# nilsfriess/ParMGMC

Measured on AMD Instinct MI355X. Metric: Gaussian samples/sec on 512^3 3D DMDA (7-pt Laplacian precision, red-black Gibbs sweep = 1 sorgibbs sample), higher is better.
Workload: dtype f64

## Files before the change

### parmgmc_amd/csrc/kernels_grid.hip

```cpp
#include <hip/hip_runtime.h>
#include <cstring>
#include <stdlib.h>
#include "pmg_kernels.h"
#define PMG_RNG_TU grid
#include "pmg_rng.hpp"

namespace {

typedef double d2 __attribute__((ext_vector_type(2)));

__device__ __forceinline__ d2 ld2(const double *p) { return *reinterpret_cast<const d2 *>(p); }

__device__ __forceinline__ d2 ld2_sys(const double *p)
{
  const unsigned long long a = __hip_atomic_load(reinterpret_cast<const unsigned long long *>(p), __ATOMIC_RELAXED, __HIP_MEMORY_SCOPE_SYSTEM);
  const unsigned long long b = __hip_atomic_load(reinterpret_cast<const unsigned long long *>(p) + 1, __ATOMIC_RELAXED, __HIP_MEMORY_SCOPE_SYSTEM);
  d2                       v;
  v.x = __longlong_as_double((long long)a);
  v.y = __longlong_as_double((long long)b);
  return v;
}
__device__ __forceinline__ void st2_sys(double *p, d2 v)
{
  __hip_atomic_store(reinterpret_cast<unsigned long long *>(p), (unsigned long long)__double_as_longlong(v.x), __ATOMIC_RELAXED, __HIP_MEMORY_SCOPE_SYSTEM);
  __hip_atomic_store(reinterpret_cast<unsigned long long *>(p) + 1, (unsigned long long)__double_as_longlong(v.y), __ATOMIC_RELAXED, __HIP_MEMORY_SCOPE_SYSTEM);
}

__device__ __forceinline__ const double *at_bytes(const double *base, uint32_t byte_off) { return reinterpret_cast<const double *>(reinterpret_cast<const char *>(base) + byte_off); }
__device__ __forceinline__ double       *at_bytes(double *base, uint32_t byte_off) { return reinterpret_cast<double *>(reinterpret_cast<char *>(base) + byte_off); }

__device__ __forceinline__ double uniform(double v)
{
  return __hiloint2double(__builtin_amdgcn_readfirstlane(__double2hiint(v)), __builtin_amdgcn_readfirstlane(__double2loint(v)));
}

template <bool PACKED>
__device__ __forceinline__ double table_at(const double (&a)[8], int idx)
{
  if (!PACKED) return uniform(a[idx]);
  double v = a[1];
  v        = idx == 2 ? a[2] : v;
  v        = idx == 3 ? a[3] : v;
  v        = idx == 4 ? a[4] : v;
  v        = idx == 5 ? a[5] : v;
  v        = idx == 6 ? a[6] : v;
  return v;
}

__device__ __forceinline__ void wave_wait_flag(const uint64_t *f, uint64_t v, unsigned *err, unsigned long long *spin_total)
{
  if (threadIdx.x == 0) {
    unsigned long long spins = 0;
    while (__hip_atomic_load(f, __ATOMIC_RELAXED, __HIP_MEMORY_SCOPE_SYSTEM) < v) {
      __builtin_amdgcn_s_sleep(8);
      ++spins;
      if ((spins & 0xFFFFu) == 0 && err && __hip_atomic_load(err, __ATOMIC_RELAXED, __HIP_MEMORY_SCOPE_SYSTEM)) break;
      if (spins > (1ull << 28)) {
        if (err) {
          err[1] = 0x10u;
          err[2] = (unsigned)v;
          err[3] = (unsigned)__hip_atomic_load(f, __ATOMIC_RELAXED, __HIP_MEMORY_SCOPE_SYSTEM);
          __hip_atomic_store(err, 1u, __ATOMIC_RELAXED, __HIP_MEMORY_SCOPE_SYSTEM);
        }
        break;
      }
    }
    if (spins && spin_total) atomicAdd(spin_total, spins);
  }
  __builtin_amdgcn_fence(__ATOMIC_ACQUIRE, "workgroup");
}

template <bool NOISY, bool OMEGA1, bool HALO, bool PACKED>
__device__ __forceinline__ void grid_color_sweep_body(const pmgk_grid_layout &L, const pmgk_grid_op &op, int c, int t, int j, int k, pmg::LogTabEntry *tab, pmg::LogTabEntry tab_entry, const pmgk_grid_halo &halo, const double *__restrict__ b_own, const double *__restrict__ y_other, double *__restrict__ y_own)
{
  const int kg = k + L.kz0;
  bool live = j < L.ny && 2 * t < L.sx && 4 * t + ((c + j + kg) & 1) < L.nx;
  if (NOISY) {
    if (!__builtin_amdgcn_ballot_w64(live)) return;
    t = live ? t : 0;
    if (PACKED) j = live ? j : 0;
  } else if (!live)
    return;
  const int p  = (c + j + kg) & 1;
  const int i0 = 4 * t + p, i1 = i0 + 2;
  const bool v1 = i1 < L.nx;

  const bool    hasS = j > 0, hasN = j < L.ny - 1, hasD = kg > 0, hasU = kg < L.nzg - 1;
  const double  h2 = op.h2;
  const int64_t  rowoff = (int64_t)(k + 1) * L.sp + (int64_t)j * L.sx;
  const uint32_t lo     = 16u * (uint32_t)t;
  const double  *yo_row = y_other + rowoff;
  const int    eo = p ? (2 * t + 2 < L.sx ? 2 : 1) : (t > 0 ? -1 : 0);
  const bool   hasW0 = i0 > 0, hasE0 = i0 < L.nx - 1, hasE1 = i1 < L.nx - 1;
  const int    nyz = PACKED ? (int)hasS + (int)hasN + (int)hasD + (int)hasU : min(j, 1) + min(L.ny - 1 - j, 1) + min(kg, 1) + min(L.nzg - 1 - kg, 1);
  const bool   two0 = hasW0 && hasE0, two1 = hasE1;
  const double idA = table_at<PACKED>(op.idiag, nyz + 1), idB = table_at<PACKED>(op.idiag, nyz + 2);
  const double sqA = NOISY ? table_at<PACKED>(op.sqrtdiag, nyz + 1) : 0.0, sqB = NOISY ? table_at<PACKED>(op.sqrtdiag, nyz + 2) : 0.0;
  double      *out_row = y_own + rowoff;
  d2     Vc = ld2(at_bytes(yo_row, lo));
  double ed = *at_bytes(yo_row, lo + 8u * (uint32_t)eo);
  d2     oS = ld2(at_bytes(yo_row - (hasS ? L.sx : 0), lo));
  d2     oN = ld2(at_bytes(yo_row + (hasN ? L.sx : 0), lo));
  const int64_t inplane = (int64_t)j * L.sx + 2 * t;
  d2      oD = (HALO && k == 0 && halo.glo) ? ld2_sys(halo.glo + inplane) : ld2(at_bytes(yo_row - (hasD ? L.sp : 0), lo));
  d2      oU = (HALO && k == L.nz - 1 && halo.ghi) ? ld2_sys(halo.ghi + inplane) : ld2(at_bytes(yo_row + (hasU ? L.sp : 0), lo));
#ifndef PMG_GRID_NO_NT
  d2     bb = __builtin_nontemporal_load(reinterpret_cast<const d2 *>(at_bytes(b_own + rowoff, lo)));
#else
  d2     bb = ld2(at_bytes(b_own + rowoff, lo));
#endif
  pmg::RngConsts K;
  if (NOISY) {
    __builtin_amdgcn_sched_barrier(0);
    K = pmg::load_sincos_consts();
    __builtin_amdgcn_sched_barrier(0);
  }

  double z0 = 0.0, z1 = 0.0;
  if (NOISY) {
    pmg::normal_pair_fill((uint32_t)t, (uint32_t)(j + (int64_t)L.ny * kg), (uint32_t)op.sweep, ((uint32_t)(op.sweep >> 32) & 0x7fffffffu) | ((uint32_t)c << 31), op.key0, op.key1, tab_entry, tab, (int)threadIdx.x, K, z0, z1);
    asm volatile("" : "+v"(Vc.x), "+v"(Vc.y), "+v"(ed), "+v"(oS.x), "+v"(oS.y), "+v"(oN.x), "+v"(oN.y), "+v"(oD.x), "+v"(oD.y), "+v"(oU.x), "+v"(oU.y), "+v"(bb.x), "+v"(bb.y) : "v"(z0), "v"(z1));
  }
  const double L0 = p ? Vc.x : ed, R0 = p ? Vc.y : Vc.x, L1 = R0, R1 = p ? ed : Vc.y;
  const double idg0 = two0 ? idB : idA, idg1 = two1 ? idB : idA;
  const double hS = hasS ? h2 : 0.0, hN = hasN ? h2 : 0.0, hD = hasD ? h2 : 0.0, hU = hasU ? h2 : 0.0;

  double w0 = bb.x, w1 = bb.y;
  if (NOISY) {
    const double sq0 = two0 ? sqB : sqA, sq1 = two1 ? sqB : sqA;
    w0 = z0 * sq0 + bb.x;
    w1 = z1 * sq1 + bb.y;
  }
  double s0 = w0, s1 = w1;
  s0 = s0 + hD * oD.x;
  s1 = s1 + hD * oD.y;
  s0 = s0 + hS * oS.x;
  s1 = s1 + hS * oS.y;
  s0 = s0 + (hasW0 ? h2 : 0.0) * L0;
  s1 = s1 + h2 * L1;
  s0 = s0 + (hasE0 ? h2 : 0.0) * R0;
  s1 = s1 + (hasE1 ? h2 : 0.0) * R1;
  s0 = s0 + hN * oN.x;
  s1 = s1 + hN * oN.y;
  s0 = s0 + hU * oU.x;
  s1 = s1 + hU * oU.y;

  double r0, r1;
  if (OMEGA1) {
    r0 = idg0 * s0;
    r1 = idg1 * s1;
  } else {
    const d2 yo2 = ld2(at_bytes(out_row, lo));
    r0           = op.one_minus_omega * yo2.x + idg0 * s0;
    r1           = op.one_minus_omega * yo2.y + idg1 * s1;
  }
  const d2 out = {r0, v1 ? r1 : 0.0};
  if (NOISY) {
    asm volatile("" ::"v"(out.x), "v"(out.y), "s"(out_row));
    if (!live) return;
  }
#ifndef PMG_GRID_NO_NT
  __builtin_nontemporal_store(out, reinterpret_cast<d2 *>(at_bytes(out_row, lo)));
#else
  *reinterpret_cast<d2 *>(at_bytes(out_row, lo)) = out;
#endif
  if (HALO) {
    if (k == 0 && halo.plo) st2_sys(halo.plo + inplane, out);
    if (k == L.nz - 1 && halo.phi) st2_sys(halo.phi + inplane, out);
  }
}

template <bool NOISY, bool OMEGA1>
__device__ __forceinline__ d2 grid_row_update(const pmgk_grid_op &op, int p, bool hasW0, bool hasE0, bool hasE1, bool v1, bool hasS, bool hasN, bool hasD, bool hasU, double h2, bool two0, bool two1, double idA, double idB, double sqA, double sqB, d2 Vc, double ed, d2 oS, d2 oN, d2 oD, d2 oU, d2 bb, double z0, double z1, const double *out_row, uint32_t lo)
{
  const double L0 = p ? Vc.x : ed, R0 = p ? Vc.y : Vc.x, L1 = R0, R1 = p ? ed : Vc.y;
  const double idg0 = two0 ? idB : idA, idg1 = two1 ? idB : idA;
  const double hS = hasS ? h2 : 0.0, hN = hasN ? h2 : 0.0, hD = hasD ? h2 : 0.0, hU = hasU ? h2 : 0.0;

  double w0 = bb.x, w1 = bb.y;
  if (NOISY) {
    const double sq0 = two0 ? sqB : sqA, sq1 = two1 ? sqB : sqA;
    w0 = z0 * sq0 + bb.x;
    w1 = z1 * sq1 + bb.y;
  }
  double s0 = w0, s1 = w1;
  s0 = s0 + hD * oD.x;
  s1 = s1 + hD * oD.y;
  s0 = s0 + hS * oS.x;
  s1 = s1 + hS * oS.y;
  s0 = s0 + (hasW0 ? h2 : 0.0) * L0;
  s1 = s1 + h2 * L1;
  s0 = s0 + (hasE0 ? h2 : 0.0) * R0;
  s1 = s1 + (hasE1 ? h2 : 0.0) * R1;
  s0 = s0 + hN * oN.x;
  s1 = s1 + hN * oN.y;
  s0 = s0 + hU * oU.x;
  s1 = s1 + hU * oU.y;

  double r0, r1;
  if (OMEGA1) {
    r0 = idg0 * s0;
    r1 = idg1 * s1;
  } else {
    const d2 yo2 = ld2(at_bytes(out_row, lo));
    r0           = op.one_minus_omega * yo2.x + idg0 * s0;
    r1           = op.one_minus_omega * yo2.y + idg1 * s1;
  }
  const d2 out = {r0, v1 ? r1 : 0.0};
  return out;
}

template <bool PACKED>
__device__ __forceinline__ void grid_thread_position(int nbx, int bandw, int ty, int &t, int &j)
{
  if (PACKED) {
    const int flat = ((int)blockIdx.x * 4 + ty) * 64 + (int)threadIdx.x;
    j              = flat / nbx;
    t              = flat - j * nbx;
  } else {
    const int bx = bandw > 0 ? (int)(blockIdx.x >> 3) : (int)blockIdx.x;
    const int jl = (int)blockIdx.y * 4 + ty;
    t            = bx * 64 + threadIdx.x;
    j            = bandw > 0 ? (jl < bandw ? (int)(blockIdx.x & 7u) * bandw + jl : 0x40000000) : jl;
  }
}

template <bool NOISY, bool OMEGA1, bool HALO, bool PACKED, bool TAIL>
__global__ __launch_bounds__(256) __attribute__((amdgpu_num_sgpr(96))) void grid_color_sweep_kernel(pmgk_grid_layout L, pmgk_grid_op op, int c, int nbx, int zmain, int bandw, int kbegin, int kstride, int kcount, int tmain, int tailw, pmgk_grid_halo halo, const double *__restrict__ b_own, const double *__restrict__ y_other, double *__restrict__ y_own)
{
  const int ty = __builtin_amdgcn_readfirstlane(threadIdx.y);
  __shared__ pmg::LogTabEntry s_logtab[NOISY ? 4 * PMG_LOGTAB_SIZE : 1];
  pmg::LogTabEntry           *tab = s_logtab + (NOISY ? ty * PMG_LOGTAB_SIZE : 0);
  pmg::LogTabEntry            tab_entry = {0.0, 0.0};
  if (NOISY) {
    const d2 e = ld2(reinterpret_cast<const double *>(pmg::g_logtab + threadIdx.x));
    tab_entry  = {e.x, e.y};
  }
  int                         t, j;
  const int                   zsplit = zmain > 0 ? zmain : kcount;
  if (TAIL && (int)blockIdx.z >= zsplit) {
    const int tb  = (int)blockIdx.x + (int)gridDim.x * ((int)blockIdx.y + (int)gridDim.y * ((int)blockIdx.z - zsplit));
    const bool compact = tailw == 1 && L.nx == 4 * tmain + 1 && (L.sx & 15) != 0;
    const int  slots   = compact ? (L.ny + 1) / 2 : L.ny * tailw;
    const int  per     = (slots + 255) / 256;
    const int  kz = tb / per, part = tb - kz * per;
    if (kz >= kcount) return;
    const int f = (part * 4 + ty) * 64 + (int)threadIdx.x, kt = kbegin + kz * kstride;
    if (compact) {
      j = 2 * f + ((c + kt + L.kz0) & 1);
      t = tmain;
    } else {
      j = f / tailw;
      t = tmain + f - j * tailw;
    }
    grid_color_sweep_body<NOISY, OMEGA1, false, true>(L, op, c, t, j, kt, tab, tab_entry, halo, b_own, y_other, y_own);
    return;
  }
  grid_thread_position<PACKED>(nbx, bandw, ty, t, j);

  int k = kbegin + (int)blockIdx.z * kstride;
  if (!HALO && !PACKED && zmain > 0) {
    const int xcd = (int)(blockIdx.x & 7u), extra = max(xcd - (8 - (L.ny - 8 * bandw)), 0);
    const int first = xcd * bandw + extra, nl = bandw + (xcd >= 8 - (L.ny - 8 * bandw) ? 1 : 0);
    const int w     = ((int)blockIdx.y + (int)gridDim.y * (int)blockIdx.z) * 4 + ty;
    if (nl <= 0) return;
    const int kz = w / nl;
    if (kz >= kcount) return;
    t = (int)(blockIdx.x >> 3) * 64 + (int)threadIdx.x;
    j = first + (w - kz * nl);
    k = kbegin + kz * kstride;
  }
  if (HALO && halo.full) {
    const int z = (int)blockIdx.z;
    k           = z == 0 ? 0 : (z == 1 ? L.nz - 1 : z - 1);
    const bool face_lo = k == 0, face_hi = k == L.nz - 1;
    if (face_lo && halo.wlo) wave_wait_flag(halo.wlo, halo.wval, halo.err, halo.spins);
    if (face_hi && halo.whi) wave_wait_flag(halo.whi, halo.wval, halo.err, halo.spins);
    grid_color_sweep_body<NOISY, OMEGA1, HALO, PACKED>(L, op, c, t, j, k, tab, tab_entry, halo, b_own, y_other, y_own);
    if (face_lo || face_hi) {
      asm volatile("s_waitcnt vmcnt(0)" ::: "memory");
      __builtin_amdgcn_fence(__ATOMIC_RELEASE, "workgroup");
      __syncthreads();
      if (threadIdx.x == 0 && threadIdx.y == 0) {
        const unsigned nface  = L.nz > 1 ? 2u : 1u;
        const unsigned expect = gridDim.x * gridDim.y * nface;
        if (atomicAdd(halo.counter, 1u) == expect - 1u) {
          *halo.counter = 0;
          if (halo.slo) __hip_atomic_store(halo.slo, halo.sval, __ATOMIC_RELAXED, __HIP_MEMORY_SCOPE_SYSTEM);
          if (halo.shi) __hip_atomic_store(halo.shi, halo.sval, __ATOMIC_RELAXED, __HIP_MEMORY_SCOPE_SYSTEM);
        }
      }
    }
    return;
  }
  grid_color_sweep_body<NOISY, OMEGA1, HALO, PACKED>(L, op, c, t, j, k, tab, tab_entry, halo, b_own, y_other, y_own);
}

struct grid_pair_launch {
  int32_t  nx, ny, sx, kz0, nzg;
  int32_t  c, kbegin, kcount, npair;
  int32_t  bandw;
  int32_t  flat;
  int32_t  thr;
  uint32_t mul0, mul1;
  uint32_t sp8, sx8;
};

template <bool OMEGA1>
__global__ __launch_bounds__(256) __attribute__((amdgpu_num_sgpr(96), amdgpu_waves_per_eu(4, 4))) void grid_color_pair_sweep_kernel(grid_pair_launch P, const double *__restrict__ b_own, const double *__restrict__ y_other, double *__restrict__ y_own, pmgk_grid_op op)
{
  const int ty = __builtin_amdgcn_readfirstlane(threadIdx.y);
  __shared__ pmg::LogTabEntry s_logtab[4 * PMG_LOGTAB_SIZE];
  pmg::LogTabEntry           *tab       = s_logtab + ty * PMG_LOGTAB_SIZE;
  const d2                    tab_e     = ld2(reinterpret_cast<const double *>(pmg::g_logtab + threadIdx.x));
  const pmg::LogTabEntry      tab_entry = {tab_e.x, tab_e.y};
  asm volatile("" ::"s"(P.sp8), "s"(P.sx8), "s"(b_own), "s"(y_other), "s"(op.key0), "s"(op.key1), "s"(op.sweep));
  const int xcd = (int)(blockIdx.x & 7u);
  int       bx, j, kz;
  if (P.flat) {
    const int  over  = xcd - P.thr;
    const int  first = xcd * P.bandw + max(over, 0), nl = P.bandw + (over >= 0 ? 1 : 0);
    const int  w     = ((int)blockIdx.y * 4 + P.flat * (int)blockIdx.z) + ty;
    kz = (int)__umulhi((uint32_t)w, over >= 0 ? P.mul1 : P.mul0);
    bx = (int)(blockIdx.x >> 3);
    j  = first + (w - kz * nl);
  } else {
    const int jl = (int)blockIdx.y * 4 + ty;
    bx = P.bandw > 0 ? (int)(blockIdx.x >> 3) : (int)blockIdx.x;
    j  = P.bandw > 0 ? (jl < P.bandw ? xcd * P.bandw + jl : 0x40000000) : jl;
    kz = (int)blockIdx.z;
  }
  if (j >= P.ny || kz >= P.npair) return;

  const bool pair = 2 * kz + 1 < P.kcount;
  const int  k0 = P.kbegin + 2 * kz, kg0 = k0 + P.kz0, kg1 = kg0 + (pair ? 1 : 0);
  const int  p0 = (P.c + j + kg0) & 1, p1 = (P.c + j + kg1) & 1;
  int        t  = bx * 64 + (int)threadIdx.x;
  const bool inrow = 2 * t < P.sx, live0 = inrow && 4 * t + p0 < P.nx, live1 = pair && inrow && 4 * t + p1 < P.nx;
  const bool live = live0 || live1;
  if (!__builtin_amdgcn_ballot_w64(live)) return;
  t = live ? t : 0;
  const bool hasS = j > 0, hasN = j < P.ny - 1, hasD0 = kg0 > 0, hasU0 = kg0 < P.nzg - 1, hasU1 = kg1 < P.nzg - 1;
  const uint32_t sp8 = P.sp8, sx8 = P.sx8, dS = hasS ? sx8 : 0u, dN = hasN ? sx8 : 0u;
  const uint32_t d0 = sp8, d1 = sp8 + (pair ? sp8 : 0u);
  const uint64_t rowm = (uint64_t)(uint32_t)k0 * sp8 + (uint32_t)j * sx8;
  const char    *yo   = reinterpret_cast<const char *>(y_other) + rowm, *bo = reinterpret_cast<const char *>(b_own) + rowm;
  const uint32_t lo   = 16u * (uint32_t)t;
  const uint32_t v0 = lo + d0, v1 = lo + d1;
  const uint32_t eW = t > 0 ? (uint32_t)-8 : 0u, eE = 2 * t + 2 < P.sx ? 16u : 8u;
  const uint32_t m0 = (uint32_t)-p0, m1 = (uint32_t)-p1;
  const uint32_t e0 = (eE & m0) | (eW & ~m0), e1 = (eE & m1) | (eW & ~m1);
  const double *yod = reinterpret_cast<const double *>(yo), *bod = reinterpret_cast<const double *>(bo);
  d2     rA  = ld2(at_bytes(yod, lo + (hasD0 ? 0u : sp8)));
  d2     rB  = ld2(at_bytes(yod, v0));
  d2     rC  = ld2(at_bytes(yod, v0 + (hasU0 ? sp8 : 0u)));
  d2     rE  = ld2(at_bytes(yod, v1 + (hasU1 ? sp8 : 0u)));
  double ed0 = *at_bytes(yod, v0 + e0);
  double ed1 = *at_bytes(yod, v1 + e1);
  d2     oS0 = ld2(at_bytes(yod, lo + (d0 - dS)));
  d2     oN0 = ld2(at_bytes(yod, lo + (d0 + dN)));
  d2     oS1 = ld2(at_bytes(yod, lo + (d1 - dS)));
  d2     oN1 = ld2(at_bytes(yod, lo + (d1 + dN)));
#ifndef PMG_GRID_NO_NT
  d2     bb0 = __builtin_nontemporal_load(reinterpret_cast<const d2 *>(at_bytes(bod, v0)));
  d2     bb1 = __builtin_nontemporal_load(reinterpret_cast<const d2 *>(at_bytes(bod, v1)));
#else
  d2     bb0 = ld2(at_bytes(bod, v0));
  d2     bb1 = ld2(at_bytes(bod, v1));
#endif
  __builtin_amdgcn_sched_barrier(0);
  int      jr = j, kr0 = kg0, kr1 = kg1;
  uint32_t key0 = op.key0, key1 = op.key1, sweep_lo = (uint32_t)op.sweep, sweep_hi = (uint32_t)(op.sweep >> 32);
  asm volatile("" : "+s"(jr), "+s"(kr0), "+s"(kr1), "+s"(key0), "+s"(key1), "+s"(sweep_lo), "+s"(sweep_hi));
  const pmg::RngConsts K = pmg::load_sincos_consts();
  const int      nyz0 = min(jr, 1) + min(P.ny - 1 - jr, 1) + min(kr0, 1) + min(P.nzg - 1 - kr0, 1);
  const int      nyz1 = min(jr, 1) + min(P.ny - 1 - jr, 1) + min(kr1, 1) + min(P.nzg - 1 - kr1, 1);
  const double   idA0 = uniform(op.idiag[nyz0 + 1]), idB0 = uniform(op.idiag[nyz0 + 2]), idA1 = uniform(op.idiag[nyz1 + 1]), idB1 = uniform(op.idiag[nyz1 + 2]);
  const double   sqA0 = uniform(op.sqrtdiag[nyz0 + 1]), sqB0 = uniform(op.sqrtdiag[nyz0 + 2]);
  const double   sqA1 = uniform(op.sqrtdiag[nyz1 + 1]), sqB1 = uniform(op.sqrtdiag[nyz1 + 2]);
  double        *out = reinterpret_cast<double *>(reinterpret_cast<char *>(y_own) + rowm);
  __builtin_amdgcn_sched_barrier(0);
  double z00, z01, z10, z11;
  pmg::normal_pair_fill2((uint32_t)t, (uint32_t)(jr + (int64_t)P.ny * kr0), (uint32_t)(jr + (int64_t)P.ny * kr1), sweep_lo, (sweep_hi & 0x7fffffffu) | ((uint32_t)P.c << 31), key0, key1, tab_entry, tab, (int)threadIdx.x, K, z00, z01, z10, z11);
  asm volatile("" : "+v"(rA.x), "+v"(rA.y), "+v"(rB.x), "+v"(rB.y), "+v"(rC.x), "+v"(rC.y), "+v"(rE.x), "+v"(rE.y), "+v"(ed0), "+v"(ed1) : "v"(z00), "v"(z01), "v"(z10), "v"(z11));
  asm volatile("" : "+v"(oS0.x), "+v"(oS0.y), "+v"(oN0.x), "+v"(oN0.y), "+v"(oS1.x), "+v"(oS1.y), "+v"(oN1.x), "+v"(oN1.y), "+v"(bb0.x), "+v"(bb0.y), "+v"(bb1.x), "+v"(bb1.y) : "v"(z00), "v"(z01), "v"(z10), "v"(z11));
  int    tr = t;
  double h2 = op.h2;
  asm volatile("" : "+v"(tr), "+s"(h2), "+s"(jr), "+s"(kr0), "+s"(kr1) : "v"(z00), "v"(z01), "v"(z10), "v"(z11));
  const bool uS = jr > 0, uN = jr < P.ny - 1, uD0 = kr0 > 0, uU0 = kr0 < P.nzg - 1, uD1 = kr1 > 0, uU1 = kr1 < P.nzg - 1;
  const int  q0 = (P.c + jr + kr0) & 1, q1 = (P.c + jr + kr1) & 1;
  const int  i00 = 4 * tr + q0, i01 = i00 + 2, i10 = 4 * tr + q1, i11 = i10 + 2;
  const bool hasW00 = i00 > 0, hasE00 = i00 < P.nx - 1, hasE01 = i01 < P.nx - 1, hasW10 = i10 > 0, hasE10 = i10 < P.nx - 1, hasE11 = i11 < P.nx - 1;
  const d2 r0 = grid_row_update<true, OMEGA1>(op, q0, hasW00, hasE00, hasE01, i01 < P.nx, uS, uN, uD0, uU0, h2, hasW00 && hasE00, hasE01, idA0, idB0, sqA0, sqB0, rB, ed0, oS0, oN0, rA, rC, bb0, z00, z01, out, v0);
  const d2 r1 = grid_row_update<true, OMEGA1>(op, q1, hasW10, hasE10, hasE11, i11 < P.nx, uS, uN, uD1, uU1, h2, hasW10 && hasE10, hasE11, idA1, idB1, sqA1, sqB1, rC, ed1, oS1, oN1, rB, rE, bb1, z10, z11, out, v1);
  asm volatile("" ::"v"(r0.x), "v"(r0.y), "v"(r1.x), "v"(r1.y), "s"(out));
#ifndef PMG_GRID_NO_NT
  if (live0) __builtin_nontemporal_store(r0, reinterpret_cast<d2 *>(at_bytes(out, v0)));
  if (live1) __builtin_nontemporal_store(r1, reinterpret_cast<d2 *>(at_bytes(out, v1)));
#else
  if (live0) *reinterpret_cast<d2 *>(at_bytes(out, v0)) = r0;
  if (live1) *reinterpret_cast<d2 *>(at_bytes(out, v1)) = r1;
#endif
}

__global__ void grid_to_cvec_kernel(pmgk_grid_layout L, const double *__restrict__ nat, double *__restrict__ cv)
{
  const int i = blockIdx.x * blockDim.x + threadIdx.x;
  const int j = blockIdx.y * blockDim.y + threadIdx.y;
  const int k = blockIdx.z;
  if (i >= L.nx || j >= L.ny) return;
  const int c = (i + j + k + L.kz0) & 1;
  cv[(int64_t)c * L.cs + (int64_t)(k + 1) * L.sp + (int64_t)j * L.sx + (i >> 1)] = nat[i + (int64_t)L.nx * (j + (int64_t)L.ny * k)];
}

__global__ void grid_from_cvec_kernel(pmgk_grid_layout L, const double *__restrict__ cv, double *__restrict__ nat)
{
  const int i = blockIdx.x * blockDim.x + threadIdx.x;
  const int j = blockIdx.y * blockDim.y + threadIdx.y;
  const int k = blockIdx.z;
  if (i >= L.nx || j >= L.ny) return;
  const int c = (i + j + k + L.kz0) & 1;
  nat[i + (int64_t)L.nx * (j + (int64_t)L.ny * k)] = cv[(int64_t)c * L.cs + (int64_t)(k + 1) * L.sp + (int64_t)j * L.sx + (i >> 1)];
}

struct residual_consts {
  double a, dA, dB, aS, aN, aD, aU;
};

__device__ __forceinline__ d2 residual_pair(const residual_consts &K, bool hasW0, bool hasE0, bool hasE1, bool v1, d2 oD, d2 oS, d2 oN, d2 oU, double L0, double R0, double L1, double R1, d2 yy, d2 bb)
{
  const double dg0 = (hasW0 && hasE0) ? K.dB : K.dA, dg1 = hasE1 ? K.dB : K.dA;
  double       s0 = 0.0, s1 = 0.0;
  s0 = s0 + K.aD * oD.x;
  s1 = s1 + K.aD * oD.y;
  s0 = s0 + K.aS * oS.x;
  s1 = s1 + K.aS * oS.y;
  s0 = s0 + (hasW0 ? K.a : 0.0) * L0;
  s1 = s1 + K.a * L1;
  s0 = s0 + dg0 * yy.x;
  s1 = s1 + dg1 * yy.y;
  s0 = s0 + (hasE0 ? K.a : 0.0) * R0;
  s1 = s1 + (hasE1 ? K.a : 0.0) * R1;
  s0 = s0 + K.aN * oN.x;
  s1 = s1 + K.aN * oN.y;
  s0 = s0 + K.aU * oU.x;
  s1 = s1 + K.aU * oU.y;
  const d2 out = {bb.x - s0, v1 ? bb.y - s1 : 0.0};
  return out;
}

template <bool PACKED>
__device__ __forceinline__ void grid_residual_values(const pmgk_grid_layout &L, const pmgk_grid_op &op, int t, int j, int k, const double *__restrict__ b, const double *__restrict__ y, int64_t &offa, int64_t &offb, d2 &outA, d2 &outB)
{
  const int      kg   = k + L.kz0;
  const int      ca   = (j + kg) & 1;
  const bool     hasS = j > 0, hasN = j < L.ny - 1, hasD = kg > 0, hasU = kg < L.nzg - 1;
  const int64_t  rowoff = (int64_t)(k + 1) * L.sp + (int64_t)j * L.sx;
  const uint32_t lo     = 16u * (uint32_t)t;
  offa = (int64_t)ca * L.cs + rowoff;
  offb = (int64_t)(1 - ca) * L.cs + rowoff;
  const double  *ya = y + offa, *yb = y + offb;
  const int64_t  dS = hasS ? L.sx : 0, dN = hasN ? L.sx : 0, dD = hasD ? L.sp : 0, dU = hasU ? L.sp : 0;
  const d2       Ya = ld2(at_bytes(ya, lo)), Yb = ld2(at_bytes(yb, lo));
  const double   edA = *at_bytes(yb, lo - (t > 0 ? 8u : 0u));
  const double   edB = *at_bytes(ya, lo + (2 * t + 2 < L.sx ? 16u : 8u));
  const int      nyz = (int)hasS + (int)hasN + (int)hasD + (int)hasU;
  residual_consts K;
  K.a  = -op.h2;
  K.dA = table_at<PACKED>(op.diag, nyz + 1);
  K.dB = table_at<PACKED>(op.diag, nyz + 2);
  K.aS = hasS ? K.a : 0.0;
  K.aN = hasN ? K.a : 0.0;
  K.aD = hasD ? K.a : 0.0;
  K.aU = hasU ? K.a : 0.0;
  const int i0 = 4 * t;
  outA = residual_pair(K, i0 > 0, i0 < L.nx - 1, i0 + 2 < L.nx - 1, i0 + 2 < L.nx, ld2(at_bytes(yb - dD, lo)), ld2(at_bytes(yb - dS, lo)), ld2(at_bytes(yb + dN, lo)), ld2(at_bytes(yb + dU, lo)), edA, Yb.x, Yb.x, Yb.y, Ya, ld2(at_bytes(b + offa, lo)));
  outB = d2{0.0, 0.0};
  if (i0 + 1 < L.nx)
    outB = residual_pair(K, true, i0 + 1 < L.nx - 1, i0 + 3 < L.nx - 1, i0 + 3 < L.nx, ld2(at_bytes(ya - dD, lo)), ld2(at_bytes(ya - dS, lo)), ld2(at_bytes(ya + dN, lo)), ld2(at_bytes(ya + dU, lo)), Ya.x, Ya.y, Ya.y, edB, Yb, ld2(at_bytes(b + offb, lo)));
}

template <bool PACKED>
__device__ __forceinline__ void grid_residual_body(const pmgk_grid_layout &L, const pmgk_grid_op &op, int t, int j, int k, const double *__restrict__ b, const double *__restrict__ y, double *__restrict__ r)
{
  if (j >= L.ny || 2 * t >= L.sx || 4 * t >= L.nx) return;
  int64_t offa, offb;
  d2      outA, outB;
  grid_residual_values<PACKED>(L, op, t, j, k, b, y, offa, offb, outA, outB);
  const uint32_t lo = 16u * (uint32_t)t;
  *reinterpret_cast<d2 *>(at_bytes(r + offa, lo)) = outA;
  if (4 * t + 1 < L.nx) *reinterpret_cast<d2 *>(at_bytes(r + offb, lo)) = outB;
}

__device__ __forceinline__ double lane_prev_d(double v)
{
  return __hiloint2double(__builtin_amdgcn_update_dpp(0, __double2hiint(v), 0x138, 0xf, 0xf, false), __builtin_amdgcn_update_dpp(0, __double2loint(v), 0x138, 0xf, 0xf, false));
}
__device__ __forceinline__ double lane_next_d(double v)
{
  return __hiloint2double(__builtin_amdgcn_update_dpp(0, __double2hiint(v), 0x130, 0xf, 0xf, false), __builtin_amdgcn_update_dpp(0, __double2loint(v), 0x130, 0xf, 0xf, false));
}

struct rr_acc {
  double s0, s1;
};
struct rr_thread {
  int      t, J0;
  uint32_t lo;
  bool     left, right0, right1;
  bool     eW0, eE0, eE1, eV1;
  bool     oE0, oE1, oV1, ovalid;
};

__device__ __forceinline__ void rr_add(rr_acc &a, double wyz, const rr_thread &T, double Lf, const d2 &E, const d2 &O)
{
  const double h = 0.5 * wyz;
  a.s0 = a.s0 + (T.left ? h : 0.0) * Lf;
  a.s0 = a.s0 + wyz * E.x;
  a.s0 = a.s0 + (T.right0 ? h : 0.0) * O.x;
  a.s1 = a.s1 + h * O.x;
  a.s1 = a.s1 + wyz * E.y;
  a.s1 = a.s1 + (T.right1 ? h : 0.0) * O.y;
}

struct rr_line {
  d2 ev, od;
};

struct rr_planes {
  const double *v, *lo2, *hi2;
  int           kz0, nz;
  uint32_t      sp8, cs8;
};
struct rr_plane {
  const double *p;
  uint32_t      base, cst;
};
__device__ __forceinline__ rr_plane rr_plane_of(const rr_planes &P, int g)
{
  const int kl = g - P.kz0;
  rr_plane  r;
  if (kl >= -1 && kl <= P.nz) {
    r.p    = P.v;
    r.base = (uint32_t)(kl + 1) * P.sp8;
    r.cst  = P.cs8;
  } else {
    r.p    = kl < 0 ? P.lo2 : P.hi2;
    r.base = 0;
    r.cst  = P.sp8;
  }
  return r;
}

__device__ __forceinline__ rr_line rr_load_line(const rr_plane &pl, uint32_t line, int parity)
{
  const uint32_t c = parity ? pl.cst : 0u;
  rr_line        r;
  r.ev = ld2(at_bytes(pl.p, pl.base + line + c));
  r.od = ld2(at_bytes(pl.p, pl.base + line + (pl.cst - c)));
  return r;
}

template <bool SYNC>
__global__ __launch_bounds__(256) void grid_residual_restrict_kernel(pmgk_grid_layout L, pmgk_grid_op op, pmgk_st27_dims C, int tplE, int wpp, int kc, int nchunks, const double *__restrict__ b, const double *__restrict__ y, const double *__restrict__ ylo2, const double *__restrict__ yhi2, double *__restrict__ bc)
{
  const int xcd = (int)blockIdx.x & 7, q = (int)blockIdx.x >> 3, per = (int)gridDim.x >> 3;
  const int gw  = __builtin_amdgcn_readfirstlane((xcd * per + q) * 4 + (int)(threadIdx.x >> 6));
  const int wppb = SYNC ? (wpp + 3) / 4 * 4 : wpp;
  const int zc = gw / wppb, wv = gw - zc * wppb;
  if (zc >= nchunks) return;
  const int  lane = threadIdx.x & 63, nslots = C.ny * tplE;
  const int  fu = 62 * wv + lane - 1, f = min(max(fu, 0), nslots - 1);
  const bool store = lane >= 1 && lane <= 62 && fu < nslots;
  rr_thread  T;
  const int  Jc = f / tplE;
  T.t      = f - Jc * tplE;
  T.J0     = Jc;
  T.lo     = 16u * (uint32_t)T.t;
  const int i0 = 4 * T.t, I0 = 2 * T.t;
  T.left   = I0 > 0;
  T.right0 = i0 + 1 < L.nx;
  T.right1 = i0 + 3 < L.nx;
  T.eW0    = i0 > 0;
  T.eE0    = i0 < L.nx - 1;
  T.eE1    = i0 + 2 < L.nx - 1;
  T.eV1    = i0 + 2 < L.nx;
  T.oE0    = i0 + 1 < L.nx - 1;
  T.oE1    = i0 + 3 < L.nx - 1;
  T.oV1    = i0 + 3 < L.nx;
  T.ovalid = i0 + 1 < L.nx;
  const int      K0 = C.kz0 + zc * kc, K1 = min(K0 + kc, C.kz0 + C.nz);
  const int      kfirst = max(2 * K0 - 1, 0), klast = min(2 * K1 - 1, L.nzg - 1), jmax = L.ny - 1;
  const uint32_t sx8 = 8u * (uint32_t)L.sx;
  const rr_planes PY = {y, ylo2, yhi2, L.kz0, L.nz, 8u * (uint32_t)L.sp, 8u * (uint32_t)L.cs};
  const rr_planes PB = {b, b, b, L.kz0, L.nz, 8u * (uint32_t)L.sp, 8u * (uint32_t)L.cs};
  const double   ma = -op.h2;
  rr_acc         a = {0.0, 0.0}, n = {0.0, 0.0};
  double        *out = bc + I0 + (int64_t)C.nx * (Jc + (int64_t)C.ny * (K0 - C.kz0 + 1));
  const int64_t  cplane = (int64_t)C.nx * C.ny;
  rr_line        Dv[3], Cv[3], Uv[3], hS, hN;
  {
    const int      kd = max(kfirst - 1, 0);
    const rr_plane pd = rr_plane_of(PY, kd), pc = rr_plane_of(PY, kfirst);
#pragma unroll
    for (int i = 0; i < 3; ++i) {
      const int      jc = min(max(2 * Jc - 1 + i, 0), jmax);
      const uint32_t ln = (uint32_t)jc * sx8 + T.lo;
      Dv[i] = rr_load_line(pd, ln, (jc + kd) & 1);
      Cv[i] = rr_load_line(pc, ln, (jc + kfirst) & 1);
    }
    const int jS = min(max(2 * Jc - 2, 0), jmax), jN = min(max(2 * Jc + 2, 0), jmax);
    hS = rr_load_line(pc, (uint32_t)jS * sx8 + T.lo, (jS + kfirst) & 1);
    hN = rr_load_line(pc, (uint32_t)jN * sx8 + T.lo, (jN + kfirst) & 1);
  }
  for (int k = kfirst; k <= klast; ++k) {
    if (SYNC) __syncthreads();
    int J = Jc;
    asm volatile("" : "+v"(J));
    const bool     hasD = k > 0, hasU = k < L.nzg - 1, odd = k & 1;
    const int      nzc = (int)hasD + (int)hasU, ku = hasU ? k + 1 : k;
    const double   dg2 = uniform(op.diag[nzc + 2]), dg3 = uniform(op.diag[nzc + 3]), dg4 = uniform(op.diag[nzc + 4]);
    const double   wz = odd ? 0.5 : 1.0;
    const rr_plane pu = rr_plane_of(PY, ku), pb = rr_plane_of(PB, k);
    const int      jS = min(max(2 * J - 2, 0), jmax), jN = min(max(2 * J + 2, 0), jmax);
#ifdef PMG_RR_PROBE_IDEAL
    (void)jS;
    (void)jN;
#pragma unroll
    for (int i = 1; i < 3; ++i) {
      const int      jc = min(max(2 * J - 1 + i, 0), jmax);
      Uv[i] = rr_load_line(pu, (uint32_t)jc * sx8 + T.lo, (jc + ku) & 1);
    }
    Uv[0] = Uv[2];
    const rr_line hSu = Uv[1], hNu = Uv[1];
#else
    const rr_line  hSu = rr_load_line(pu, (uint32_t)jS * sx8 + T.lo, (jS + ku) & 1);
    const rr_line  hNu = rr_load_line(pu, (uint32_t)jN * sx8 + T.lo, (jN + ku) & 1);
#pragma unroll
    for (int i = 0; i < 3; ++i) {
      const int      jc = min(max(2 * J - 1 + i, 0), jmax);
      Uv[i] = rr_load_line(pu, (uint32_t)jc * sx8 + T.lo, (jc + ku) & 1);
    }
#endif
#pragma unroll
    for (int i = 0; i < 3; ++i) {
      const int      j = 2 * J - 1 + i, jc = min(max(j, 0), jmax);
#ifdef PMG_RR_PROBE_IDEAL
      const int      jb = min(max(2 * J - 1 + (i == 0 ? 2 : i), 0), jmax);
      const rr_line  bb = rr_load_line(pb, (uint32_t)jb * sx8 + T.lo, (jb + k) & 1);
#else
      const rr_line  bb = rr_load_line(pb, (uint32_t)jc * sx8 + T.lo, (jc + k) & 1);
#endif
      const rr_line &S = i == 0 ? hS : Cv[i > 0 ? i - 1 : 0], &N = i == 2 ? hN : Cv[i < 2 ? i + 1 : 2];
      const bool     hasS = jc > 0, hasN = jc < jmax, inner = hasS && hasN;
      residual_consts Kc;
      Kc.a  = ma;
      Kc.dA = inner ? dg3 : dg2;
      Kc.dB = inner ? dg4 : dg3;
      Kc.aS = hasS ? ma : 0.0;
      Kc.aN = hasN ? ma : 0.0;
      Kc.aD = hasD ? ma : 0.0;
      Kc.aU = hasU ? ma : 0.0;
      const double edA = lane_prev_d(Cv[i].od.y), edB = lane_next_d(Cv[i].ev.x);
      const d2     E = residual_pair(Kc, T.eW0, T.eE0, T.eE1, T.eV1, Dv[i].ev, S.ev, N.ev, Uv[i].ev, edA, Cv[i].od.x, Cv[i].od.x, Cv[i].od.y, Cv[i].ev, bb.ev);
      d2           O = residual_pair(Kc, true, T.oE0, T.oE1, T.oV1, Dv[i].od, S.od, N.od, Uv[i].od, Cv[i].ev.x, Cv[i].ev.y, Cv[i].ev.y, edB, Cv[i].od, bb.od);
      if (!T.ovalid) O = d2{0.0, 0.0};
      const double Lf = lane_prev_d(O.y);
      const double w  = ((unsigned)j < (unsigned)L.ny) ? (i == 1 ? wz : 0.5 * wz) : 0.0;
      rr_add(a, w, T, Lf, E, O);
      if (odd) rr_add(n, w, T, Lf, E, O);
    }
    if (odd) {
      if (k > 2 * K0 - 1) {
        if (store) {
          out[0] = a.s0;
          if (I0 + 1 < C.nx) out[1] = a.s1;
        }
        out += cplane;
      }
      a = n;
      n = rr_acc{0.0, 0.0};
    }
#pragma unroll
    for (int i = 0; i < 3; ++i) {
      Dv[i] = Cv[i];
      Cv[i] = Uv[i];
    }
    hS = hSu;
    hN = hNu;
  }
  if (2 * K1 - 1 > klast && store) {
    out[0] = a.s0;
    if (I0 + 1 < C.nx) out[1] = a.s1;
  }
}

template <bool PACKED, bool TAIL>
__global__ __launch_bounds__(256) void grid_residual_kernel(pmgk_grid_layout L, pmgk_grid_op op, int bandw, int tplE, int tmain, int tailw, const double *__restrict__ b, const double *__restrict__ y, double *__restrict__ r)
{
  const int ty = __builtin_amdgcn_readfirstlane(threadIdx.y);
  if (TAIL && (int)blockIdx.z >= L.nz) {
    const int tb  = (int)blockIdx.x + (int)gridDim.x * ((int)blockIdx.y + (int)gridDim.y * ((int)blockIdx.z - L.nz));
    const int per = (L.ny * tailw + 255) / 256;
    const int kz = tb / per, part = tb - kz * per;
    if (kz >= L.nz) return;
    const int f = (part * 4 + ty) * 64 + (int)threadIdx.x, j = f / tailw;
    grid_residual_body<true>(L, op, tmain + f - j * tailw, j, kz, b, y, r);
    return;
  }
  int t, j;
  grid_thread_position<PACKED>(tplE, bandw, ty, t, j);
  grid_residual_body<PACKED>(L, op, t, j, (int)blockIdx.z, b, y, r);
}

inline int launch_status() { return hipGetLastError() == hipSuccess ? 0 : 1; }

}

static inline int grid_threads_per_line(const pmgk_grid_layout *L) { return ((L->nx + 1) / 2 + 1) / 2; }
static inline bool grid_use_packed(const pmgk_grid_layout *L)
{
  static int env = -1;
  if (env < 0) {
    const char *e = getenv("PMG_GRID_PACKED");
    env           = e ? atoi(e) : 2;
  }
  if (env != 2) return env == 1;
  const int tplE = grid_threads_per_line(L), lanes = (L->sx / 2 + 63) / 64 * 64;
  return 2 * lanes >= 3 * tplE;
}

static const char *const grid_plane_pair_key = "PMG_GRID_PLANE_PAIR";

struct grid_mapping {
  bool packed, tail, pair;
  int  nbx, nby, bandw, tmain, tailw, ztail, zmain;
  dim3 grid;
};

static grid_mapping grid_choose_mapping(const pmgk_grid_layout *L, int kcount, bool allow_tail, bool allow_flat = false, bool allow_pair = false)
{
  const int kcount_planes = kcount;
  static int banded_env = -1, tail_env = -1, flat_env = -1, pair_env = -1;
  if (banded_env < 0) {
    const char *e = getenv("PMG_GRID_BANDED");
    banded_env    = e ? atoi(e) : 1;
    e             = getenv("PMG_GRID_TAIL");
    tail_env      = e ? atoi(e) : 1;
    e             = getenv("PMG_GRID_FLAT");
    flat_env      = e ? atoi(e) : 1;
    e             = getenv(grid_plane_pair_key);
    pair_env      = e ? atoi(e) : 1;
  }
  grid_mapping M;
  const int    tpl = L->sx / 2, tplE = grid_threads_per_line(L);
  M.nby   = (L->ny + 3) / 4;
  M.tmain = tplE / 64 * 64;
  M.tailw = tplE - M.tmain;
  M.tail   = allow_tail && tail_env && M.tmain > 0 && M.tailw > 0 && M.tailw <= 8;
  M.packed = !M.tail && grid_use_packed(L);
  M.nbx    = M.packed ? tplE : (M.tail ? M.tmain / 64 : (tpl + 63) / 64);
  M.bandw = (!M.packed && banded_env && M.nby >= 16) ? (L->ny + 7) / 8 : 0;
  M.ztail = 0;
  M.zmain = 0;
  M.pair = allow_pair && pair_env && !M.packed && !M.tail && (M.bandw == 0 || kcount >= 4);
  if (M.pair) kcount = (kcount + 1) / 2;
  if (M.packed) M.grid = dim3((unsigned)(((int64_t)L->ny * tplE + 255) / 256), 1, kcount);
  else {
    const unsigned gx = M.bandw > 0 ? 8 * M.nbx : M.nbx, gy = M.bandw > 0 ? (M.bandw + 3) / 4 : M.nby;
    if (allow_flat && flat_env && M.bandw > 0 && ((M.bandw & 3) || 8 * M.bandw != L->ny)) {
      M.bandw           = L->ny / 8;
      const int maxband = M.bandw + (L->ny > 8 * M.bandw ? 1 : 0);
      M.zmain           = (int)(((int64_t)maxband * kcount + 4 * gy - 1) / (4 * gy));
    }
    const int zlayers = M.zmain > 0 ? M.zmain : kcount;
    if (M.tail) {
      const int64_t nblocks = (int64_t)kcount * (((int64_t)L->ny * M.tailw + 255) / 256);
      M.ztail               = (int)((nblocks + (int64_t)gx * gy - 1) / ((int64_t)gx * gy));
    }
    M.grid = dim3(gx, gy, zlayers + M.ztail);
  }
  if (!M.tail) M.tmain = M.tailw = 0;
  if (M.pair && (8 * (3 * L->sp + 2 * (int64_t)L->sx) >= ((int64_t)1 << 32) || (M.zmain > 0 && (M.bandw < 2 || 4 * (int64_t)M.grid.y * M.grid.z * (M.bandw + 1) >= ((int64_t)1 << 32)))))
    return grid_choose_mapping(L, kcount_planes, allow_tail, allow_flat, false);
  return M;
}

static grid_pair_launch grid_pair_constants(const grid_mapping &M, const pmgk_grid_layout &L, int color, int kbegin, int kcount)
{
  grid_pair_launch P;
  P.nx     = L.nx;
  P.ny     = L.ny;
  P.sx     = L.sx;
  P.kz0    = L.kz0;
  P.nzg    = L.nzg;
  P.c      = color;
  P.kbegin = kbegin;
  P.kcount = kcount;
  P.npair  = (kcount + 1) >> 1;
  P.bandw  = M.bandw;
  P.flat   = M.zmain > 0 ? 4 * (int)M.grid.y : 0;
  P.thr    = 8 - (L.ny - 8 * M.bandw);
  P.mul0   = M.zmain > 0 ? (uint32_t)((((uint64_t)1 << 32) + M.bandw - 1) / M.bandw) : 0u;
  P.mul1   = M.zmain > 0 ? (uint32_t)((((uint64_t)1 << 32) + M.bandw) / (M.bandw + 1)) : 0u;
  P.sp8    = (uint32_t)(8 * L.sp);
  P.sx8    = 8u * (uint32_t)L.sx;
  return P;
}

template <bool NOISY, bool OMEGA1, bool HALO>
static void launch_sweep(const grid_mapping &M, dim3 block, hipStream_t s, const pmgk_grid_layout &L, const pmgk_grid_op &op, int color, int kbegin, int kstride, int kcount, const pmgk_grid_halo &h, const double *bo, const double *yo, double *ys)
{
  if (M.packed) hipLaunchKernelGGL((grid_color_sweep_kernel<NOISY, OMEGA1, HALO, true, false>), M.grid, block, 0, s, L, op, color, M.nbx, 0, M.bandw, kbegin, kstride, kcount, 0, 0, h, bo, yo, ys);
  else if (!HALO && M.tail) hipLaunchKernelGGL((grid_color_sweep_kernel<NOISY, OMEGA1, false, false, true>), M.grid, block, 0, s, L, op, color, M.nbx, M.zmain, M.bandw, kbegin, kstride, kcount, M.tmain, M.tailw, h, bo, yo, ys);
  else {
    if constexpr (NOISY && !HALO) {
      if (M.pair) {
        hipLaunchKernelGGL((grid_color_pair_sweep_kernel<OMEGA1>), M.grid, block, 0, s, grid_pair_constants(M, L, color, kbegin, kcount), bo, yo, ys, op);
        return;
      }
    }
    hipLaunchKernelGGL((grid_color_sweep_kernel<NOISY, OMEGA1, HALO, false, false>), M.grid, block, 0, s, L, op, color, M.nbx, HALO ? 0 : M.zmain, M.bandw, kbegin, kstride, kcount, 0, 0, h, bo, yo, ys);
  }
}

extern "C" int pmgk_grid_color_sweep(const pmgk_grid_layout *L, const pmgk_grid_op *op, int color, int kbegin, int kcount, int kstride, const pmgk_grid_halo *halo, const double *b, double *y, void *stream)
{
  if (kcount <= 0) return 0;
  const grid_mapping M = grid_choose_mapping(L, kcount, !halo, !halo, !halo && kstride == 1 && op->noisy);
  const dim3         block(64, 4, 1);
  hipStream_t   s  = (hipStream_t)stream;
  const double *bo = b + (int64_t)color * L->cs, *yo = y + (int64_t)(1 - color) * L->cs;
  double       *ys = y + (int64_t)color * L->cs;
  pmgk_grid_halo h0;
  memset(&h0, 0, sizeof h0);
  if (halo) {
    if (op->noisy) {
      if (op->omega_is_one) launch_sweep<true, true, true>(M, block, s, *L, *op, color, kbegin, kstride, kcount, *halo, bo, yo, ys);
      else launch_sweep<true, false, true>(M, block, s, *L, *op, color, kbegin, kstride, kcount, *halo, bo, yo, ys);
    } else {
      if (op->omega_is_one) launch_sweep<false, true, true>(M, block, s, *L, *op, color, kbegin, kstride, kcount, *halo, bo, yo, ys);
      else launch_sweep<false, false, true>(M, block, s, *L, *op, color, kbegin, kstride, kcount, *halo, bo, yo, ys);
    }
  } else if (op->noisy) {
    if (op->omega_is_one) launch_sweep<true, true, false>(M, block, s, *L, *op, color, kbegin, kstride, kcount, h0, bo, yo, ys);
    else launch_sweep<true, false, false>(M, block, s, *L, *op, color, kbegin, kstride, kcount, h0, bo, yo, ys);
  } else {
    if (op->omega_is_one) launch_sweep<false, true, false>(M, block, s, *L, *op, color, kbegin, kstride, kcount, h0, bo, yo, ys);
    else launch_sweep<false, false, false>(M, block, s, *L, *op, color, kbegin, kstride, kcount, h0, bo, yo, ys);
  }
  return launch_status();
}

extern "C" int pmgk_grid_residual(const pmgk_grid_layout *L, const pmgk_grid_op *op, const double *b, const double *y, double *r, void *stream)
{
  if (L->nz <= 0) return 0;
  const grid_mapping M = grid_choose_mapping(L, L->nz, true);
  const dim3         block(64, 4, 1);
  const int          tplE = grid_threads_per_line(L);
  if (M.packed) hipLaunchKernelGGL((grid_residual_kernel<true, false>), M.grid, block, 0, (hipStream_t)stream, *L, *op, M.bandw, tplE, 0, 0, b, y, r);
  else if (M.tail) hipLaunchKernelGGL((grid_residual_kernel<false, true>), M.grid, block, 0, (hipStream_t)stream, *L, *op, M.bandw, tplE, M.tmain, M.tailw, b, y, r);
  else hipLaunchKernelGGL((grid_residual_kernel<false, false>), M.grid, block, 0, (hipStream_t)stream, *L, *op, M.bandw, tplE, 0, 0, b, y, r);
  return launch_status();
}

extern "C" int pmgk_grid_residual_restrict_applies(const pmgk_grid_layout *L, const pmgk_st27_dims *C, int have_lo2, int have_hi2)
{
  static const int off  = getenv("PMG_GRID_FUSED_RR") ? !atoi(getenv("PMG_GRID_FUSED_RR")) : 0;
  const int        tplE = grid_threads_per_line(L);
  const bool       slab = L->kz0 != 0 || L->nz != L->nzg;
  if (off || C->nz <= 0) return 0;
  if (!slab && (C->kz0 != 0 || C->nz != C->nzg)) return 0;
  if (slab && ((L->kz0 > 0 && !have_lo2) || (L->kz0 + L->nz < L->nzg && !have_hi2) || L->nz < 2)) return 0;
  if (L->nx < 3 || L->ny < 3 || L->nzg < 3 || !(L->nx & 1) || !(L->ny & 1) || !(L->nzg & 1)) return 0;
  if (C->nx != (L->nx + 1) / 2 || C->ny != (L->ny + 1) / 2 || C->nzg != (L->nzg + 1) / 2) return 0;
  if (tplE != (C->nx + 1) / 2 || (int64_t)C->ny * tplE >= ((int64_t)1 << 30)) return 0;
  if (2 * (int64_t)L->cs * 8 >= ((int64_t)1 << 32)) return 0;
  if (slab && (2 * C->kz0 < L->kz0 || 2 * (C->kz0 + C->nz - 1) >= L->kz0 + L->nz)) return 0;
  return 1;
}

extern "C" int pmgk_grid_residual_restrict(const pmgk_grid_layout *L, const pmgk_grid_op *op, const pmgk_st27_dims *C, const double *b, const double *y, const double *ylo2, const double *yhi2, double *bc, void *stream)
{
  static const int kc_env = getenv("PMG_GRID_RR_CHUNK") ? atoi(getenv("PMG_GRID_RR_CHUNK")) : 0;
  if (!pmgk_grid_residual_restrict_applies(L, C, ylo2 != nullptr, yhi2 != nullptr)) return -1;
  const int     tplE = grid_threads_per_line(L);
  static const int sync_knob = getenv("PMG_GRID_RR_SYNC") ? atoi(getenv("PMG_GRID_RR_SYNC")) : -1;
  const int        sync_env  = sync_knob >= 0 ? sync_knob : ((int64_t)L->nx * L->ny * L->nz >= 8000000);
  const int     wpp = (int)(((int64_t)C->ny * tplE + 61) / 62);
  int           kc  = kc_env > 0 ? kc_env : 8;
  while (kc_env <= 0 && kc > 2 && (int64_t)wpp * ((C->nz + kc - 1) / kc) < 2048) kc >>= 1;
  const int     nchunks = (C->nz + kc - 1) / kc;
  if (sync_env) {
    const int64_t nblocks = (int64_t)((wpp + 3) / 4) * nchunks;
    hipLaunchKernelGGL(grid_residual_restrict_kernel<true>, dim3((unsigned)((nblocks + 7) / 8 * 8)), dim3(256), 0, (hipStream_t)stream, *L, *op, *C, tplE, wpp, kc, nchunks, b, y, ylo2, yhi2, bc);
  } else {
    const int64_t nblocks = ((int64_t)wpp * nchunks + 3) / 4;
    hipLaunchKernelGGL(grid_residual_restrict_kernel<false>, dim3((unsigned)((nblocks + 7) / 8 * 8)), dim3(256), 0, (hipStream_t)stream, *L, *op, *C, tplE, wpp, kc, nchunks, b, y, ylo2, yhi2, bc);
  }
  return launch_status();
}

extern "C" int pmgk_grid_to_cvec(const pmgk_grid_layout *L, const double *nat, double *cvec, void *stream)
{
  const dim3 block(64, 4, 1);
  const dim3 grid((L->nx + 63) / 64, (L->ny + 3) / 4, L->nz);
  hipLaunchKernelGGL(grid_to_cvec_kernel, grid, block, 0, (hipStream_t)stream, *L, nat, cvec);
  return launch_status();
}

extern "C" int pmgk_grid_from_cvec(const pmgk_grid_layout *L, const double *cvec, double *nat, void *stream)
{
  const dim3 block(64, 4, 1);
  const dim3 grid((L->nx + 63) / 64, (L->ny + 3) / 4, L->nz);
  hipLaunchKernelGGL(grid_from_cvec_kernel, grid, block, 0, (hipStream_t)stream, *L, cvec, nat);
  return launch_status();
}
```

Baseline: 1750.

## Add 4x4 y-z tile sweep kernel sharing neighbor rows through LDS

Adds a new noisy red-black sweep kernel where each 64x4 block handles 4 consecutive z-planes for 4 y-rows. Each thread keeps a 6-plane column of the other color in registers, and the north/south neighbors are exchanged through shared memory. This replaces redundant global loads of the stencil neighbours used by the plane-pair kernel. It is enabled by default when the pair path applies, ny is a multiple of 32 and kcount is at least 8. The cost is extra LDS use, a block barrier, and fixed waves-per-EU and SGPR limits that may restrict occupancy.

```diff
diff --git a/parmgmc_amd/csrc/kernels_grid.hip b/parmgmc_amd/csrc/kernels_grid.hip
--- a/parmgmc_amd/csrc/kernels_grid.hip
+++ b/parmgmc_amd/csrc/kernels_grid.hip
@@ -403,6 +403,107 @@
 #endif
 }
 
+struct grid_tile_launch {
+  int32_t  nx, ny, sx, kz0, nzg;
+  int32_t  c, kbegin, kcount;
+  int32_t  bandw;
+  uint32_t sp8, sx8;
+};
+
+template <bool OMEGA1>
+__global__ __launch_bounds__(256) __attribute__((amdgpu_num_sgpr(96), amdgpu_waves_per_eu(4, 4))) void grid_color_tile_sweep_kernel(grid_tile_launch P, const double *__restrict__ b_own, const double *__restrict__ y_other, double *__restrict__ y_own, pmgk_grid_op op)
+{
+  const int ty = __builtin_amdgcn_readfirstlane(threadIdx.y);
+  __shared__ pmg::LogTabEntry s_logtab[4 * PMG_LOGTAB_SIZE];
+  __shared__ d2               s_rows[4][6][64];
+  pmg::LogTabEntry           *tab       = s_logtab + ty * PMG_LOGTAB_SIZE;
+  const d2                    tab_e     = ld2(reinterpret_cast<const double *>(pmg::g_logtab + threadIdx.x));
+  const pmg::LogTabEntry      tab_entry = {tab_e.x, tab_e.y};
+  asm volatile("" ::"s"(P.sp8), "s"(P.sx8), "s"(b_own), "s"(y_other), "s"(op.key0), "s"(op.key1), "s"(op.sweep));
+  const int  lane = (int)threadIdx.x;
+  const int  j0   = (int)(blockIdx.x & 7u) * P.bandw + 4 * (int)blockIdx.y, j = j0 + ty;
+  const int  k0   = P.kbegin + 4 * (int)blockIdx.z, klast = P.kbegin + P.kcount - 1;
+  int        t    = (int)(blockIdx.x >> 3) * 64 + lane;
+  const bool inrow = 2 * t < P.sx;
+  t                = inrow ? t : 0;
+  const int  plo = -P.kz0, phi = min(P.nzg - 1 - P.kz0, klast + 1);
+  const uint32_t sp8 = P.sp8, sx8 = P.sx8;
+  uint32_t dR[6];
+#pragma unroll
+  for (int r = 0; r < 6; ++r) dR[r] = (uint32_t)(min(max(k0 + r - 1, plo), phi) - (k0 - 1)) * sp8;
+  uint32_t dQ[4];
+#pragma unroll
+  for (int q = 0; q < 4; ++q) dQ[q] = (uint32_t)(min(k0 + q, klast) - (k0 - 1)) * sp8;
+  const uint64_t rowm = (uint64_t)(uint32_t)k0 * sp8 + (uint32_t)j * sx8;
+  const double  *yod  = reinterpret_cast<const double *>(reinterpret_cast<const char *>(y_other) + rowm);
+  const double  *bod  = reinterpret_cast<const double *>(reinterpret_cast<const char *>(b_own) + rowm);
+  const uint32_t lo   = 16u * (uint32_t)t;
+  const uint32_t dX  = (uint32_t)(min(max(k0 + ty, plo), phi) - (k0 - 1)) * sp8;
+  const uint32_t dXS = dX - (uint32_t)(j - max(j0 - 1, 0)) * sx8, dXN = dX + (uint32_t)(min(j0 + 4, P.ny - 1) - j) * sx8;
+  const uint32_t eW = t > 0 ? (uint32_t)-8 : 0u, eE = 2 * t + 2 < P.sx ? 16u : 8u;
+  const int      pj = P.c + j + P.kz0;
+  d2     R[6];
+  double ed[4];
+  d2     bb[4];
+#pragma unroll
+  for (int r = 1; r < 5; ++r) R[r] = ld2(at_bytes(yod, lo + dR[r]));
+  d2 xS = ld2(at_bytes(yod, lo + dXS));
+  d2 xN = ld2(at_bytes(yod, lo + dXN));
+  R[0]  = ld2(at_bytes(yod, lo + dR[0]));
+  R[5]  = ld2(at_bytes(yod, lo + dR[5]));
+#pragma unroll
+  for (int q = 0; q < 4; ++q) {
+    const uint32_t m = (uint32_t) - ((pj + min(k0 + q, klast)) & 1);
+    ed[q]            = *at_bytes(yod, lo + dQ[q] + ((eE & m) | (eW & ~m)));
+  }
+#pragma unroll
+  for (int q = 0; q < 4; ++q) bb[q] = __builtin_nontemporal_load(reinterpret_cast<const d2 *>(at_bytes(bod, lo + dQ[q])));
+  __builtin_amdgcn_sched_barrier(0);
+  int      jr = j, kr = k0;
+  uint32_t key0 = op.key0, key1 = op.key1, sweep_lo = (uint32_t)op.sweep, sweep_hi = (uint32_t)(op.sweep >> 32);
+  asm volatile("" : "+s"(jr), "+s"(kr), "+s"(key0), "+s"(key1), "+s"(sweep_lo), "+s"(sweep_hi));
+  const pmg::RngConsts K = pmg::load_sincos_consts();
+  __builtin_amdgcn_sched_barrier(0);
+  int kg[4];
+#pragma unroll
+  for (int q = 0; q < 4; ++q) kg[q] = min(kr + q, klast) + P.kz0;
+  double z[4][2];
+  const uint32_t c3 = (sweep_hi & 0x7fffffffu) | ((uint32_t)P.c << 31);
+  pmg::normal_pair_fill2((uint32_t)t, (uint32_t)(jr + (int64_t)P.ny * kg[0]), (uint32_t)(jr + (int64_t)P.ny * kg[1]), sweep_lo, c3, key0, key1, tab_entry, tab, lane, K, z[0][0], z[0][1], z[1][0], z[1][1]);
+  pmg::normal_pair_fill2((uint32_t)t, (uint32_t)(jr + (int64_t)P.ny * kg[2]), (uint32_t)(jr + (int64_t)P.ny * kg[3]), sweep_lo, c3, key0, key1, tab_entry, tab, lane, K, z[2][0], z[2][1], z[3][0], z[3][1]);
+#pragma unroll
+  for (int r = 0; r < 6; ++r) asm volatile("" : "+v"(R[r].x), "+v"(R[r].y) : "v"(z[0][0]), "v"(z[1][0]), "v"(z[2][0]), "v"(z[3][0]));
+  asm volatile("" : "+v"(xS.x), "+v"(xS.y), "+v"(xN.x), "+v"(xN.y) : "v"(z[0][1]), "v"(z[1][1]), "v"(z[2][1]), "v"(z[3][1]));
+  const int    nj = min(jr, 1) + min(P.ny - 1 - jr, 1);
+  double       h2 = op.h2;
+  double       id1 = uniform(op.idiag[nj + 2]), id2 = uniform(op.idiag[nj + 3]), id3 = uniform(op.idiag[nj + 4]);
+  double       sq1 = uniform(op.sqrtdiag[nj + 2]), sq2 = uniform(op.sqrtdiag[nj + 3]), sq3 = uniform(op.sqrtdiag[nj + 4]);
+#pragma unroll
+  for (int q = 0; q < 4; ++q) s_rows[q][ty + 1][lane] = R[q + 1];
+  s_rows[ty][0][lane] = xS;
+  s_rows[ty][5][lane] = xN;
+  asm volatile("" : "+s"(h2), "+s"(id1), "+s"(id2), "+s"(id3), "+s"(sq1), "+s"(sq2), "+s"(sq3));
+  __syncthreads();
+  d2 oS[4], oN[4];
+#pragma unroll
+  for (int q = 0; q < 4; ++q) {
+    oS[q] = s_rows[q][ty][lane];
+    oN[q] = s_rows[q][ty + 2][lane];
+  }
+  double    *out = reinterpret_cast<double *>(reinterpret_cast<char *>(y_own) + rowm);
+  const bool uS = jr > 0, uN = jr < P.ny - 1;
+#pragma unroll
+  for (int q = 0; q < 4; ++q) {
+    const bool   uD = kg[q] > 0, uU = kg[q] < P.nzg - 1, face = !(uD && uU);
+    const double idA = face ? id1 : id2, idB = face ? id2 : id3, sqA = face ? sq1 : sq2, sqB = face ? sq2 : sq3;
+    const int    pq  = (P.c + jr + kg[q]) & 1;
+    const int    i0 = 4 * t + pq, i1 = i0 + 2;
+    const bool   hasW0 = i0 > 0, hasE0 = i0 < P.nx - 1, hasE1 = i1 < P.nx - 1;
+    const d2     r = grid_row_update<true, OMEGA1>(op, pq, hasW0, hasE0, hasE1, i1 < P.nx, uS, uN, uD, uU, h2, hasW0 && hasE0, hasE1, idA, idB, sqA, sqB, R[q + 1], ed[q], oS[q], oN[q], R[q], R[q + 2], bb[q], z[q][0], z[q][1], out, lo + dQ[q]);
+    if (inrow && kr + q <= klast && i0 < P.nx) __builtin_nontemporal_store(r, reinterpret_cast<d2 *>(at_bytes(out, lo + dQ[q])));
+  }
+}
+
 __global__ void grid_to_cvec_kernel(pmgk_grid_layout L, const double *__restrict__ nat, double *__restrict__ cv)
 {
   const int i = blockIdx.x * blockDim.x + threadIdx.x;
@@ -731,9 +832,10 @@
 }
 
 static const char *const grid_plane_pair_key = "PMG_GRID_PLANE_PAIR";
+static const char *const grid_tile_key = "PMG_GRID_TILE";
 
 struct grid_mapping {
-  bool packed, tail, pair;
+  bool packed, tail, pair, tile;
   int  nbx, nby, bandw, tmain, tailw, ztail, zmain;
   dim3 grid;
 };
@@ -741,7 +843,7 @@
 static grid_mapping grid_choose_mapping(const pmgk_grid_layout *L, int kcount, bool allow_tail, bool allow_flat = false, bool allow_pair = false)
 {
   const int kcount_planes = kcount;
-  static int banded_env = -1, tail_env = -1, flat_env = -1, pair_env = -1;
+  static int banded_env = -1, tail_env = -1, flat_env = -1, pair_env = -1, tile_env = -1;
   if (banded_env < 0) {
     const char *e = getenv("PMG_GRID_BANDED");
     banded_env    = e ? atoi(e) : 1;
@@ -751,6 +853,8 @@
     flat_env      = e ? atoi(e) : 1;
     e             = getenv(grid_plane_pair_key);
     pair_env      = e ? atoi(e) : 1;
+    e             = getenv(grid_tile_key);
+    tile_env      = e ? atoi(e) : 1;
   }
   grid_mapping M;
   const int    tpl = L->sx / 2, tplE = grid_threads_per_line(L);
@@ -764,6 +868,12 @@
   M.ztail = 0;
   M.zmain = 0;
   M.pair = allow_pair && pair_env && !M.packed && !M.tail && (M.bandw == 0 || kcount >= 4);
+  M.tile = M.pair && tile_env && M.bandw > 0 && L->ny % 32 == 0 && L->ny >= 64 && kcount >= 8 && 8 * (5 * L->sp + 5 * (int64_t)L->sx) < ((int64_t)1 << 32);
+  if (M.tile) {
+    M.grid = dim3(8 * M.nbx, M.bandw / 4, (kcount + 3) / 4);
+    M.tmain = M.tailw = 0;
+    return M;
+  }
   if (M.pair) kcount = (kcount + 1) / 2;
   if (M.packed) M.grid = dim3((unsigned)(((int64_t)L->ny * tplE + 255) / 256), 1, kcount);
   else {
@@ -815,6 +925,22 @@
   else if (!HALO && M.tail) hipLaunchKernelGGL((grid_color_sweep_kernel<NOISY, OMEGA1, false, false, true>), M.grid, block, 0, s, L, op, color, M.nbx, M.zmain, M.bandw, kbegin, kstride, kcount, M.tmain, M.tailw, h, bo, yo, ys);
   else {
     if constexpr (NOISY && !HALO) {
+      if (M.tile) {
+        grid_tile_launch T;
+        T.nx     = L.nx;
+        T.ny     = L.ny;
+        T.sx     = L.sx;
+        T.kz0    = L.kz0;
+        T.nzg    = L.nzg;
+        T.c      = color;
+        T.kbegin = kbegin;
+        T.kcount = kcount;
+        T.bandw  = M.bandw;
+        T.sp8    = (uint32_t)(8 * L.sp);
+        T.sx8    = 8u * (uint32_t)L.sx;
+        hipLaunchKernelGGL((grid_color_tile_sweep_kernel<OMEGA1>), M.grid, block, 0, s, T, bo, yo, ys, op);
+        return;
+      }
       if (M.pair) {
         hipLaunchKernelGGL((grid_color_pair_sweep_kernel<OMEGA1>), M.grid, block, 0, s, grid_pair_constants(M, L, color, kbegin, kcount), bo, yo, ys, op);
         return;
```

Result: no change. 1767 (median of 6 runs) (+0.9%).
